# gmh14/tssplat

Hardware: AMD Instinct MI355X
Metric: tetrahedra/sec (energy fwd+bwd) (higher is better)
Workload: dtype f32

## Files before the change

### include/tssplat_amd.h

```cpp
#ifndef TSSPLAT_AMD_H
#define TSSPLAT_AMD_H

#include <stdint.h>

#ifdef __cplusplus
extern "C" {
#endif

typedef struct tsamd_handle tsamd_handle;

typedef enum tsamd_status {
    TSAMD_OK = 0,
    TSAMD_ERR_INVALID_ARGUMENT = 1,
    TSAMD_ERR_BAD_MESH = 2,
    TSAMD_ERR_NO_DEVICE = 3,
    TSAMD_ERR_HIP = 4,
    TSAMD_ERR_IO = 5,
    TSAMD_ERR_TILING = 6,
    TSAMD_ERR_HOST_ONLY = 7
} tsamd_status;

typedef struct tsamd_options {
    int32_t struct_size;
    int32_t device;
// ... 14 lines not shown
    int64_t n_tiles;
    int64_t n_components;
    int64_t total_slots;
    int64_t total_tile_vertices;
    int64_t shared_vertex_copies;
    int64_t finish_vertices;
    int64_t device_bytes;
    int32_t max_slots, max_tile_vertices, block_threads, lds_bytes;
    int32_t slots_per_thread;
    int32_t n_planes;
} tsamd_plan_info;

typedef struct tsamd_partition_info {
    int64_t owned_tets;
    int64_t halo_slots;
    int64_t staged_rows;
    int64_t n_tiles;
    int64_t tile_capacity;
    int64_t min_tiles;
    int64_t cut_components;
    int64_t bisection_components;
    int64_t cut_templates;
    double mean_fill, max_fill;
} tsamd_partition_info;

typedef struct tsamd_tile_view {
    int32_t n_slots, n_owned, s_pad, n_verts, n_excl;
    int64_t stage_off;
    int32_t n_rows;
    int32_t rec_base;
    const uint32_t *planes;
    const uint16_t *row_start;
    const int32_t *gvid;
    const int32_t *vdst;
    const int32_t *slot_tet;
    const float *rest;
} tsamd_tile_view;

const char *tsamd_last_error(void);
const char *tsamd_version(void);
#define TSAMD_ABI_VERSION 3
int32_t tsamd_abi_version(void);

int tsamd_create(const float *rest_xyz, int64_t n_vertices, const int32_t *tets, int64_t n_tets,
                 const tsamd_options *options, tsamd_handle **out);
int tsamd_create_from_veg(const char *path, const tsamd_options *options, tsamd_handle **out);
int tsamd_create_with_operator(const float *rest_xyz, int64_t n_vertices, const int32_t *tets, int64_t n_tets,
                               const int64_t *op_rowptr, const int32_t *op_col, const double *op_val,
                               const tsamd_options *options, tsamd_handle **out);
void tsamd_destroy(tsamd_handle *h);

int64_t tsamd_num_vertices(const tsamd_handle *h);
int64_t tsamd_num_tets(const tsamd_handle *h);
int tsamd_get_plan_info(const tsamd_handle *h, tsamd_plan_info *out);
int tsamd_get_partition_info(const tsamd_handle *h, tsamd_partition_info *out);
int tsamd_get_tile(const tsamd_handle *h, int64_t tile, tsamd_tile_view *out);
int tsamd_get_finish_lists(const tsamd_handle *h, int64_t *n_finish, const int32_t **vid,
                           const int32_t **off, const int32_t **idx);
int tsamd_get_adjacency(const tsamd_handle *h, const int32_t **nbr);

int tsamd_forward(tsamd_handle *h, const float *x_dev, float c1, float c2, int order,
                  void *stream, float *energy_dev);
int tsamd_backward(tsamd_handle *h, const float *x_dev, const float *grad_out_dev, float c1, float c2,
                   int order, void *stream, float *grad_dev);
int tsamd_forward_backward(tsamd_handle *h, const float *x_dev, const float *grad_out_dev, float c1,
                           float c2, int order, void *stream, float *energy_dev, float *grad_dev);
int tsamd_evaluate_dev_coef(tsamd_handle *h, const float *x_dev, const float *grad_out_dev, const float *coef_dev,
                            int order, void *stream, float *energy_dev, float *grad_dev);
typedef struct tsamd_graph tsamd_graph;
int tsamd_graph_create(tsamd_handle *h, const float *x_dev, const float *grad_out_dev, int order, float *energy_dev,
                       float *grad_dev, tsamd_graph **out);
int tsamd_graph_launch(tsamd_graph *graph, float c1, float c2, void *stream);
int tsamd_graph_launch_to(tsamd_graph *graph, float c1, float c2, void *stream, float *energy_copy_dev, float *grad_dev);
void tsamd_graph_destroy(tsamd_graph *graph);

typedef struct tsamd_train_loop tsamd_train_loop;
int64_t tsamd_train_loop_workspace_bytes(int32_t n_iters);
int tsamd_train_loop_create(tsamd_handle *h, float *param_dev, float *grad_dev, float *g1_dev, float *g2_dev, float *energy_ring_dev,
                            void *workspace_dev, int32_t n_iters, tsamd_train_loop **out);
int tsamd_train_loop_launch(tsamd_train_loop *loop, const float *c1, const float *c2, const int32_t *order, float lr, float beta1, float beta2,
                            int64_t first_step, const float *grad_limit, void *stream);
// ... 90 lines not shown
```

### tssplat_amd/_capi.py

```python
from __future__ import annotations

import ctypes as C
import os

from . import _build

_lib = None


class TsamdError(RuntimeError):

    def __init__(self, code: int, message: str):
        super().__init__(f"tssplat_amd error {code}: {message}")
        self.code = code


class Options(C.Structure):
    _fields_ = [
        ("struct_size", C.c_int32),
        ("device", C.c_int32),
        ("lds_budget_bytes", C.c_int32),
        ("max_threads", C.c_int32),
        ("target_owned", C.c_int32),
        ("lane_search_sweeps", C.c_int32),
# ... 4 lines not shown
        ("rebuild_dminv", C.c_int32),
        ("abi_version", C.c_int32),
    ]


class PlanInfo(C.Structure):
    _fields_ = [
        ("n_vertices", C.c_int64), ("n_tets", C.c_int64), ("n_tiles", C.c_int64),
        ("n_components", C.c_int64), ("total_slots", C.c_int64), ("total_tile_vertices", C.c_int64),
        ("shared_vertex_copies", C.c_int64), ("finish_vertices", C.c_int64), ("device_bytes", C.c_int64),
        ("max_slots", C.c_int32), ("max_tile_vertices", C.c_int32), ("block_threads", C.c_int32),
        ("lds_bytes", C.c_int32), ("slots_per_thread", C.c_int32), ("n_planes", C.c_int32),
    ]

    def as_dict(self) -> dict:
        return {k: int(getattr(self, k)) for k, _ in self._fields_}


class PartitionInfo(C.Structure):
    _fields_ = [
        ("owned_tets", C.c_int64), ("halo_slots", C.c_int64), ("staged_rows", C.c_int64), ("n_tiles", C.c_int64),
        ("tile_capacity", C.c_int64), ("min_tiles", C.c_int64), ("cut_components", C.c_int64),
        ("bisection_components", C.c_int64), ("cut_templates", C.c_int64), ("mean_fill", C.c_double), ("max_fill", C.c_double),
    ]


class TileView(C.Structure):
    _fields_ = [
        ("n_slots", C.c_int32), ("n_owned", C.c_int32), ("s_pad", C.c_int32), ("n_verts", C.c_int32),
        ("n_excl", C.c_int32), ("stage_off", C.c_int64), ("n_rows", C.c_int32), ("rec_base", C.c_int32),
        ("planes", C.POINTER(C.c_uint32)), ("row_start", C.POINTER(C.c_uint16)),
        ("gvid", C.POINTER(C.c_int32)), ("vdst", C.POINTER(C.c_int32)), ("slot_tet", C.POINTER(C.c_int32)), ("rest", C.POINTER(C.c_float)),
    ]


ABI_VERSION = 3

SIGNATURES = {
    "tsamd_last_error": (C.c_char_p, []),
    "tsamd_version": (C.c_char_p, []),
    "tsamd_abi_version": (C.c_int32, []),
    "tsamd_create": (C.c_int, [C.c_void_p, C.c_int64, C.c_void_p, C.c_int64, C.POINTER(Options), C.POINTER(C.c_void_p)]),
    "tsamd_create_with_operator": (C.c_int, [C.c_void_p, C.c_int64, C.c_void_p, C.c_int64, C.c_void_p, C.c_void_p, C.c_void_p,
                                             C.POINTER(Options), C.POINTER(C.c_void_p)]),
    "tsamd_create_from_veg": (C.c_int, [C.c_char_p, C.POINTER(Options), C.POINTER(C.c_void_p)]),
    "tsamd_destroy": (None, [C.c_void_p]),
    "tsamd_num_vertices": (C.c_int64, [C.c_void_p]),
    "tsamd_num_tets": (C.c_int64, [C.c_void_p]),
    "tsamd_get_plan_info": (C.c_int, [C.c_void_p, C.POINTER(PlanInfo)]),
    "tsamd_get_partition_info": (C.c_int, [C.c_void_p, C.POINTER(PartitionInfo)]),
    "tsamd_get_tile": (C.c_int, [C.c_void_p, C.c_int64, C.POINTER(TileView)]),
    "tsamd_get_finish_lists": (C.c_int, [C.c_void_p, C.POINTER(C.c_int64), C.POINTER(C.POINTER(C.c_int32)),
                                         C.POINTER(C.POINTER(C.c_int32)), C.POINTER(C.POINTER(C.c_int32))]),
    "tsamd_get_adjacency": (C.c_int, [C.c_void_p, C.POINTER(C.POINTER(C.c_int32))]),
    "tsamd_forward": (C.c_int, [C.c_void_p, C.c_void_p, C.c_float, C.c_float, C.c_int, C.c_void_p, C.c_void_p]),
    "tsamd_backward": (C.c_int, [C.c_void_p, C.c_void_p, C.c_void_p, C.c_float, C.c_float, C.c_int, C.c_void_p,
                                 C.c_void_p]),
    "tsamd_forward_backward": (C.c_int, [C.c_void_p, C.c_void_p, C.c_void_p, C.c_float, C.c_float, C.c_int,
                                         C.c_void_p, C.c_void_p, C.c_void_p]),
    "tsamd_evaluate_dev_coef": (C.c_int, [C.c_void_p, C.c_void_p, C.c_void_p, C.c_void_p, C.c_int, C.c_void_p, C.c_void_p,
                                          C.c_void_p]),
    "tsamd_graph_create": (C.c_int, [C.c_void_p, C.c_void_p, C.c_void_p, C.c_int, C.c_void_p, C.c_void_p, C.POINTER(C.c_void_p)]),
    "tsamd_graph_launch": (C.c_int, [C.c_void_p, C.c_float, C.c_float, C.c_void_p]),
    "tsamd_graph_launch_to": (C.c_int, [C.c_void_p, C.c_float, C.c_float, C.c_void_p, C.c_void_p, C.c_void_p]),
    "tsamd_graph_destroy": (None, [C.c_void_p]),
    "tsamd_read_energy_terms": (C.c_int, [C.c_void_p, C.c_void_p, C.POINTER(C.c_double)]),
    "tsamd_set_timing": (C.c_int, [C.c_void_p, C.c_int]),
    "tsamd_get_timing": (C.c_int, [C.c_void_p, C.POINTER(C.c_double), C.POINTER(C.c_double), C.POINTER(C.c_int64)]),
    "tsamd_scale": (C.c_int, [C.c_void_p, C.c_void_p, C.c_void_p, C.c_int64, C.c_void_p]),
    "tsamd_adam_uniform_step": (C.c_int, [C.c_void_p, C.c_void_p, C.c_void_p, C.c_void_p, C.c_int64, C.c_float, C.c_float,
                                        C.c_float, C.c_int64, C.c_float, C.c_void_p, C.c_void_p]),
    "tsamd_grad_limit_workspace_bytes": (C.c_int64, []),
    "tsamd_grad_limit": (C.c_int, [C.c_void_p, C.c_int64, C.c_float, C.c_float, C.c_void_p, C.c_void_p]),
    "tsamd_train_loop_workspace_bytes": (C.c_int64, [C.c_int32]),
    "tsamd_train_loop_create": (C.c_int, [C.c_void_p, C.c_void_p, C.c_void_p, C.c_void_p, C.c_void_p, C.c_void_p, C.c_void_p, C.c_int32,
                                          C.POINTER(C.c_void_p)]),
# ... 123 lines not shown
```

### tssplat_amd/csrc/capi.cpp

```cpp
#include "../../include/tssplat_amd.h"

#include <hip/hip_runtime_api.h>

#include <algorithm>
#include <cmath>
#include <cstdio>
#include <cstdlib>
#include <cstring>
#include <new>
#include <string>
#include <thread>
#include <vector>

#include "capi_common.h"
#include "kernels.h"
#include "plan.h"

namespace {

thread_local std::string g_err;

int fail(int code, const std::string &msg)
{
    g_err = msg;
    return code;
}

}

namespace tsamd {
int capi_fail(int code, const std::string &msg) { return fail(code, msg); }
}

using tsamd::DeviceGuard;

struct tsamd_handle {
    tsamd::Plan plan;
    bool host_only = true;
    int device = -1;
    int64_t device_bytes = 0;
    tsamd::TileDesc *d_tiles = nullptr;
    uint8_t *d_blob = nullptr;
    int32_t *d_gvid = nullptr, *d_vdst = nullptr, *d_fin_vid = nullptr, *d_fin_off = nullptr;
    float *d_stage = nullptr;
    double *d_partials = nullptr;
    double *d_terms = nullptr;
    float *d_energy_scratch = nullptr;
    bool timing = false;
    std::vector<hipEvent_t> events;
};

struct tsamd_graph {
    tsamd::EvalGraph *g = nullptr;
    int device = -1;
};

namespace {

template <class T>
int upload(T *&dst, const void *src, size_t count, int64_t &bytes)
{
    const size_t nbytes = (count ? count : 1) * sizeof(T);
    TSAMD_HIP(hipMalloc(reinterpret_cast<void **>(&dst), nbytes));
    if (count && src) TSAMD_HIP(hipMemcpy(dst, src, count * sizeof(T), hipMemcpyHostToDevice));
    bytes += int64_t(nbytes);
    return TSAMD_OK;
}

void release(tsamd_handle *h)
{
    if (!h) return;
    if (!h->host_only) {
        DeviceGuard g;
        (void)g.enter(h->device);
        (void)hipFree(h->d_tiles);
        (void)hipFree(h->d_blob);
        (void)hipFree(h->d_gvid);
        (void)hipFree(h->d_fin_vid);
        (void)hipFree(h->d_fin_off);
        (void)hipFree(h->d_vdst);
        (void)hipFree(h->d_stage);
        (void)hipFree(h->d_partials);
        (void)hipFree(h->d_terms);
        (void)hipFree(h->d_energy_scratch);
        for (hipEvent_t e : h->events) (void)hipEventDestroy(e);
    }
    delete h;
}

int to_device(tsamd_handle *h, int device)
{
    int count = 0;
    if (hipGetDeviceCount(&count) != hipSuccess || count <= 0)
        return fail(TSAMD_ERR_NO_DEVICE, "no HIP device is visible (this library has no CPU fallback)");
    if (device < 0) TSAMD_HIP(hipGetDevice(&device));
    if (device >= count) return fail(TSAMD_ERR_INVALID_ARGUMENT, "device ordinal out of range");
    hipDeviceProp_t prop;
    TSAMD_HIP(hipGetDeviceProperties(&prop, device));
    if (size_t(h->plan.lds_bytes) > prop.sharedMemPerBlock && size_t(h->plan.lds_bytes) > prop.maxSharedMemoryPerMultiProcessor)
        return fail(TSAMD_ERR_NO_DEVICE, std::string("device ") + prop.name + " (" + prop.gcnArchName +
                                             ") offers less LDS per workgroup than the plan needs; built for gfx950");
    DeviceGuard g;
// ... 6 lines not shown
    if (tsamd::planes_paired(P.spt) && !P.tiles.empty()) {
        tsamd::RawVector<uint32_t> image(P.blob.size());
        const int64_t T = int64_t(P.tiles.size());
        const int nthr = int(std::max<int64_t>(1, std::min<int64_t>({int64_t(std::thread::hardware_concurrency()), 64, T / 64 + 1})));
        std::vector<std::thread> pool;
        for (int w = 0; w < nthr; ++w)
            pool.emplace_back([&, w]() {
                for (int64_t t = T * w / nthr; t < T * (w + 1) / nthr; ++t) {
                    const tsamd::TileDesc &d = P.tiles[size_t(t)];
                    const size_t b0 = size_t(d.blob_off / 4), b1 = t + 1 < T ? size_t(P.tiles[size_t(t) + 1].blob_off / 4) : P.blob.size();
                    const size_t np = size_t(P.n_planes) * size_t(d.s_pad);
                    tsamd::interleave_tile_planes(P.blob.data() + b0, image.data() + b0, P.n_planes, d.s_pad, P.spt);
                    std::memcpy(image.data() + b0 + np, P.blob.data() + b0 + np, (b1 - b0 - np) * 4);
                }
            });
        for (auto &th : pool) th.join();
        const size_t head = size_t(P.tiles[0].blob_off / 4);
        if (head) std::memcpy(image.data(), P.blob.data(), head * 4);
        if ((rc = upload(h->d_blob, reinterpret_cast<const uint8_t *>(image.data()), image.size() * 4, h->device_bytes))) return rc;
    } else if ((rc = upload(h->d_blob, reinterpret_cast<const uint8_t *>(P.blob.data()), P.blob.size() * 4, h->device_bytes))) {
        return rc;
    }
    if ((rc = upload(h->d_gvid, P.gvid.data(), P.gvid.size(), h->device_bytes))) return rc;
    if ((rc = upload(h->d_vdst, P.vdst.data(), P.vdst.size(), h->device_bytes))) return rc;
    if ((rc = upload(h->d_fin_vid, P.fin_vid.data(), P.fin_vid.size(), h->device_bytes))) return rc;
    if ((rc = upload(h->d_fin_off, P.fin_off.data(), P.fin_off.size(), h->device_bytes))) return rc;
    if ((rc = upload(h->d_stage, nullptr, size_t(P.n_stage) * 3 + 3 , h->device_bytes))) return rc;
    if ((rc = upload(h->d_partials, nullptr, P.tiles.size() * 2, h->device_bytes))) return rc;
    if ((rc = upload(h->d_terms, nullptr, 2, h->device_bytes))) return rc;
    if ((rc = upload(h->d_energy_scratch, nullptr, 1, h->device_bytes))) return rc;
    TSAMD_HIP(hipMemset(h->d_terms, 0, 2 * sizeof(double)));
    {
        const hipError_t ce = tsamd::configure_kernels(P.lds_bytes);
        if (ce == hipErrorInvalidDeviceFunction)
            return fail(TSAMD_ERR_HIP, "a tile kernel of this build has a static LDS object: its dynamic LDS array no longer starts at LDS "
                                       "address 0, which the kernels' absolute LDS addressing relies on (kernels.hip: lds_at)");
        TSAMD_HIP(ce);
    }
    return TSAMD_OK;
}

int create_common(const float *rest, int64_t n, const int32_t *tets, int64_t m, const tsamd_options *o,
                  tsamd_handle **out, const tsamd::ElementOperatorCSR *op = nullptr)
{
    if (!out) return fail(TSAMD_ERR_INVALID_ARGUMENT, "out is null");
    *out = nullptr;
    tsamd_options opt;
    std::memset(&opt, 0, sizeof(opt));
    opt.device = -1;
// ... 76 lines not shown
            return rc;
        }
    }
    *out = h;
    return TSAMD_OK;
}

int check_eval(tsamd_handle *h, const float *x)
{
    if (!h) return fail(TSAMD_ERR_INVALID_ARGUMENT, "handle is null");
    if (h->host_only) return fail(TSAMD_ERR_HOST_ONLY, "handle was created host_only; no device path");
    if (!x && h->plan.n > 0) return fail(TSAMD_ERR_INVALID_ARGUMENT, "x_dev is null");
    return TSAMD_OK;
}

tsamd::EvalArgs eval_args(tsamd_handle *h, const float *x, const float *grad_out, float c1, float c2, int order, float *energy,
                          float *grad, const float *coef)
{
    tsamd::EvalArgs a;
    a.tiles = h->d_tiles;
    a.blob = h->d_blob;
    a.gvid = h->d_gvid;
    a.vdst = h->d_vdst;
    a.fin_vid = h->d_fin_vid;
    a.fin_off = h->d_fin_off;
    a.n_tiles = int64_t(h->plan.tiles.size());
    a.n_finish = int64_t(h->plan.fin_vid.size());
    a.block_threads = h->plan.block_threads;
    a.lds_bytes = h->plan.lds_bytes;
    a.vert_stride = h->plan.vert_stride;
    a.weighted = h->plan.n_planes == tsamd::kPlanesWeighted || h->plan.n_planes == tsamd::kPlanesWeightedSym;
    a.n_planes = h->plan.n_planes;
    a.rebuild = h->plan.n_planes == tsamd::kPlanesRebuild;
    a.spt = h->plan.spt;
    a.x = x;
    a.grad_out = grad_out;
    a.c1 = c1;
    a.c2 = c2;
    a.coef = coef;
    a.order = order;
    a.grad = grad;
    a.stage = h->d_stage;
    a.partials = h->d_partials;
    a.energy = energy;
    a.terms = h->d_terms;
    return a;
}

int evaluate(tsamd_handle *h, const float *x, const float *grad_out, float c1, float c2, int order, void *stream,
             float *energy, float *grad, const float *coef = nullptr)
// ... 74 lines not shown
    out->slots_per_thread = P.spt;
    out->n_planes = P.n_planes;
    return TSAMD_OK;
}

int tsamd_get_partition_info(const tsamd_handle *h, tsamd_partition_info *out)
{
    if (!h || !out) return fail(TSAMD_ERR_INVALID_ARGUMENT, "null argument");
    const tsamd::Plan &P = h->plan;
    std::memset(out, 0, sizeof(*out));
    out->owned_tets = P.m;
    out->halo_slots = P.total_slots - P.m;
    out->staged_rows = P.n_stage;
    out->n_tiles = int64_t(P.tiles.size());
    out->tile_capacity = int64_t(P.block_threads) * P.spt;
    out->min_tiles = out->tile_capacity > 0 ? (P.total_slots + out->tile_capacity - 1) / out->tile_capacity : 0;
    out->cut_components = P.n_cut_components;
    out->bisection_components = P.n_bisection_components;
    out->cut_templates = P.n_cut_templates;
    if (out->n_tiles > 0 && out->tile_capacity > 0) {
        out->mean_fill = double(P.total_slots) / (double(out->n_tiles) * double(out->tile_capacity));
        out->max_fill = double(P.max_slots) / double(out->tile_capacity);
    }
    return TSAMD_OK;
}

int tsamd_get_tile(const tsamd_handle *h, int64_t tile, tsamd_tile_view *out)
{
    if (!h || !out) return fail(TSAMD_ERR_INVALID_ARGUMENT, "null argument");
    const tsamd::Plan &P = h->plan;
    if (tile < 0 || tile >= int64_t(P.tiles.size())) return fail(TSAMD_ERR_INVALID_ARGUMENT, "tile out of range");
    const tsamd::TileDesc &d = P.tiles[size_t(tile)];
    out->n_slots = d.n_slots;
    out->n_owned = d.n_owned;
    out->s_pad = d.s_pad;
    out->n_verts = d.n_verts;
    out->n_excl = d.n_excl;
    out->stage_off = d.stage_off;
    out->n_rows = d.n_rows;
    out->rec_base = d.rec_base;
    out->planes = P.blob.data() + d.blob_off / 4;
    out->row_start = reinterpret_cast<const uint16_t *>(reinterpret_cast<const uint8_t *>(out->planes) + tsamd::tile_rowtab_offset(P.n_planes, d.s_pad));
    out->gvid = P.gvid.data() + d.vert_off;
    out->vdst = P.vdst.data() + d.vert_off;
    out->slot_tet = P.slot_tet.data() + P.slot_base[size_t(tile)];
    out->rest = P.n_planes == tsamd::kPlanesRebuild
                    ? reinterpret_cast<const float *>(reinterpret_cast<const uint8_t *>(out->planes) + tsamd::tile_rest_offset(P.n_planes, d.s_pad))
                    : nullptr;
    return TSAMD_OK;
}

int tsamd_get_finish_lists(const tsamd_handle *h, int64_t *n_finish, const int32_t **vid, const int32_t **off,
                           const int32_t **idx)
{
    if (!h || !n_finish || !vid || !off || !idx) return fail(TSAMD_ERR_INVALID_ARGUMENT, "null argument");
    *n_finish = int64_t(h->plan.fin_vid.size());
    *vid = h->plan.fin_vid.data();
    *off = h->plan.fin_off.data();
    *idx = h->plan.fin_idx.data();
    return TSAMD_OK;
}

int tsamd_get_adjacency(const tsamd_handle *h, const int32_t **nbr)
{
    if (!h || !nbr) return fail(TSAMD_ERR_INVALID_ARGUMENT, "null argument");
    *nbr = h->plan.nbr.data();
    return TSAMD_OK;
}

int tsamd_forward(tsamd_handle *h, const float *x_dev, float c1, float c2, int order, void *stream,
                  float *energy_dev)
{
    if (!energy_dev) return fail(TSAMD_ERR_INVALID_ARGUMENT, "energy_dev is null");
    return evaluate(h, x_dev, nullptr, c1, c2, order, stream, energy_dev, nullptr);
}

int tsamd_backward(tsamd_handle *h, const float *x_dev, const float *grad_out_dev, float c1, float c2, int order,
                   void *stream, float *grad_dev)
{
    if (!grad_dev && h && h->plan.n > 0) return fail(TSAMD_ERR_INVALID_ARGUMENT, "grad_dev is null");
    return evaluate(h, x_dev, grad_out_dev, c1, c2, order, stream, nullptr, grad_dev);
}

int tsamd_forward_backward(tsamd_handle *h, const float *x_dev, const float *grad_out_dev, float c1, float c2,
                           int order, void *stream, float *energy_dev, float *grad_dev)
// ... 210 lines not shown
```

### tssplat_amd/csrc/kernels.h

```cpp
#pragma once

#include <hip/hip_runtime_api.h>

#include <cstdint>

#include "plan.h"

namespace tsamd {

struct EvalArgs {
    const TileDesc *tiles;
    const uint8_t *blob;
    const int32_t *gvid, *vdst;
    const int32_t *fin_vid, *fin_off;
    int64_t n_tiles, n_finish;
    int32_t block_threads, lds_bytes;
    int32_t vert_stride = 0;
    bool rebuild = false;
    bool weighted = false;
    int32_t n_planes = 13;
    int32_t spt = kSlotsPerLane;
    const float *x;
    const float *grad_out;
    float c1, c2;
    const float *coef = nullptr;
    int order;
    float *grad;
    float *stage;
    double *partials;
    float *energy;
    double *terms;
};

hipError_t launch_eval(const EvalArgs &a, hipStream_t stream, hipEvent_t *ev = nullptr);
struct EvalGraph;
hipError_t eval_graph_create(const EvalArgs &a, EvalGraph **out);
hipError_t eval_graph_launch(EvalGraph *g, float c1, float c2, hipStream_t stream, float *energy_copy = nullptr, float *grad = nullptr);
// ... 19 lines not shown
```

### tssplat_amd/csrc/kernels.hip

```cpp
#include <hip/hip_runtime.h>

#include <vector>

#include "kernels.h"

namespace tsamd {
namespace {

constexpr int kWave = 64;

#define SLOT_FENCE() __builtin_amdgcn_sched_barrier(0)
#define STAGE_PRIORITY(n) __builtin_amdgcn_s_setprio(n)
#define UNDEF(x) asm volatile("" : "=v"(x))
typedef uint32_t v4u __attribute__((ext_vector_type(4)));
typedef uint32_t v2u __attribute__((ext_vector_type(2)));

__device__ __forceinline__ float det3(const float *F)
{
    return -F[2] * F[4] * F[6] + F[1] * F[5] * F[6] + F[2] * F[3] * F[7] - F[0] * F[5] * F[7] - F[1] * F[3] * F[8] +
           F[0] * F[4] * F[8];
}

__device__ __forceinline__ void cof3(const float *F, float *C)
{
// ... 542 lines not shown
        };
        if (64 * vb0 < td.n_verts) vertex_sums(vb0, dst_row);
        if (64 * nw < td.n_verts) {
            for (int vb = vb0 + nw; 64 * vb < td.n_verts; vb += nw)
                vertex_sums(vb, 64 * vb + lane < td.n_verts ? g_vdst[td.vert_off + 64 * vb + lane] : 0);
        }
    }
#undef t_own
}

template <bool WITH_GRAD, int BLOCK, int WPE, bool WEIGHTED = false, bool REBUILD = false, int SPT = kSlotsPerLane>
__global__ __launch_bounds__(BLOCK, WPE) void tile_energy_kernel(const KernelArgs a)
{
    const int xcd = blockIdx.x & 7, jb = blockIdx.x >> 3;
    const int tile_end = (xcd + 1) * a.tiles_per_xcd < a.n_tiles ? (xcd + 1) * a.tiles_per_xcd : a.n_tiles;
    const int tile = xcd * a.tiles_per_xcd + jb;
    if (jb >= a.tiles_per_xcd || tile >= tile_end) return;
    const int32_t gv0 = __builtin_nontemporal_load(&as_global(a.gvid)[size_t(tile) * size_t(a.vert_stride) + size_t(int(threadIdx.x) < a.vert_stride ? threadIdx.x : 0)]);
    __builtin_amdgcn_sched_barrier(0);
    tile_body<WITH_GRAD, WEIGHTED, REBUILD, SPT>(a, tile, gv0);
}

struct FinishArgs {
    const int32_t *fin_vid, *fin_off;
    int64_t n_finish;
    const float *stage;
    float *grad;
    const float *grad_out;
    const double *partials;
    int64_t n_tiles;
    float c1, c2;
    const float *coef;
    float *energy;
    double *terms;
    float *energy_copy;
};

template <int T>
__device__ __forceinline__ void energy_reduce(const FinishArgs &a, double *red)
{
    const int tid = threadIdx.x;
    const double2 *part = reinterpret_cast<const double2 *>(a.partials);
    double s = 0.0, b = 0.0;
    int64_t t = tid;
    for (; t + 7 * T < a.n_tiles; t += 8 * T) {
        double2 v[8];
#pragma unroll
// ... 25 lines not shown
        const float c1 = a.coef ? a.coef[0] : a.c1, c2 = a.coef ? a.coef[1] : a.c2;
        const float e = float(double(c1) * red[0] + double(c2) * red[T]);
        a.energy[0] = e;
        if (a.energy_copy) a.energy_copy[0] = e;
    }
}

__global__ __launch_bounds__(1024) void energy_reduce_kernel(const FinishArgs a)
{
    __shared__ double red[2 * 1024];
    energy_reduce<1024>(a, red);
}

#define FIN_LOAD(p) (*(p))
__global__ __launch_bounds__(256) void finish_kernel(const FinishArgs a)
{
    __shared__ double red[2 * 256];
    const int tid = threadIdx.x;
    if (blockIdx.x == 0) {
        if (a.energy) energy_reduce<256>(a, red);
        return;
    }
    const float gscale = a.grad_out ? *a.grad_out : 1.f;
    const int64_t stride = int64_t(gridDim.x - 1) * 256;
    for (int64_t k = int64_t(blockIdx.x - 1) * 256 + tid; k < a.n_finish; k += stride) {
        float gx = 0.f, gy = 0.f, gz = 0.f;
        const int32_t e0 = FIN_LOAD(&a.fin_off[k]), e1 = FIN_LOAD(&a.fin_off[k + 1]);
        constexpr int kRowsAhead = 4;
        {
            float3 r[kRowsAhead];
#pragma unroll
            for (int j = 0; j < kRowsAhead; ++j) {
                const int32_t e = e0 + j < e1 ? e0 + j : (e1 > 0 ? e1 - 1 : 0);
                const float *p = a.stage + size_t(e) * 3;
                r[j] = make_float3(FIN_LOAD(p), FIN_LOAD(p + 1), FIN_LOAD(p + 2));
            }
#pragma unroll
            for (int j = 0; j < kRowsAhead; ++j)
                if (e0 + j < e1) {
                    gx += r[j].x;
                    gy += r[j].y;
                    gz += r[j].z;
                }
        }
        for (int32_t e = e0 + kRowsAhead; e < e1; ++e) {
            const float *r = a.stage + size_t(e) * 3;
            gx += FIN_LOAD(r);
            gy += FIN_LOAD(r + 1);
            gz += FIN_LOAD(r + 2);
        }
        float *g = a.grad + size_t(FIN_LOAD(&a.fin_vid[k])) * 3;
        g[0] = gx * gscale;
        g[1] = gy * gscale;
        g[2] = gz * gscale;
    }
}

__global__ __launch_bounds__(256) void scale_kernel(const float *in, const float *scalar, float *out, int64_t n)
{
    const float s = *scalar;
    if (in == out && s == 1.f) return;
    const int64_t stride = int64_t(gridDim.x) * 256;
    const int64_t n4 = n >> 2;
    const float4 *in4 = reinterpret_cast<const float4 *>(in);
    float4 *out4 = reinterpret_cast<float4 *>(out);
    const bool vec = ((reinterpret_cast<uintptr_t>(in) | reinterpret_cast<uintptr_t>(out)) & 15) == 0;
    if (vec) {
        for (int64_t i = int64_t(blockIdx.x) * 256 + threadIdx.x; i < n4; i += stride) {
            float4 v = in4[i];
            out4[i] = make_float4(v.x * s, v.y * s, v.z * s, v.w * s);
        }
        for (int64_t i = 4 * n4 + int64_t(blockIdx.x) * 256 + threadIdx.x; i < n; i += stride) out[i] = in[i] * s;
    } else {
        for (int64_t i = int64_t(blockIdx.x) * 256 + threadIdx.x; i < n; i += stride) out[i] = in[i] * s;
    }
}

// ... 188 lines not shown
        k.tiles = e.tiles;
        k.blob = e.blob;
        k.gvid = e.gvid;
        k.vdst = e.vdst;
        k.x = e.x;
        k.grad_out = e.grad_out;
        k.grad = e.grad;
        k.stage = e.stage;
        k.partials = e.partials;
        set_coefficients(k, e.c1, e.c2);
        k.coef = e.coef;
        k.order = e.order;
        k.n_tiles = int(e.n_tiles);
        k.tiles_per_xcd = int((e.n_tiles + 7) / 8);
        k.vert_stride = e.vert_stride;
        k.n_planes = e.n_planes;
        r.tile_fn = tile_kernel_for(e.spt, e.block_threads, e.grad != nullptr, e.weighted, e.rebuild);
        if (!r.tile_fn) return hipErrorInvalidConfiguration;
        r.tile_block = dim3(unsigned(e.block_threads));
        r.tile_grid = dim3(unsigned(8 * k.tiles_per_xcd));
        r.tile_lds = size_t(e.lds_bytes);
    }
    FinishArgs &f = r.f;
    f.fin_vid = e.fin_vid;
    f.fin_off = e.fin_off;
    f.n_finish = e.grad ? e.n_finish : 0;
    f.stage = e.stage;
    f.grad = e.grad;
    f.grad_out = e.grad_out;
    f.partials = e.partials;
    f.n_tiles = e.n_tiles;
    f.c1 = e.c1;
    f.c2 = e.c2;
    f.coef = e.coef;
    f.energy = e.energy;
    f.terms = e.terms;
    f.energy_copy = nullptr;
    if (f.n_finish > 0) {
        r.finish_fn = reinterpret_cast<const void *>(&finish_kernel);
        r.finish_grid = dim3(1u + unsigned(grid_for(f.n_finish, 256, 1 << 20)));
        r.finish_block = dim3(256);
    } else if (f.energy) {
        r.finish_fn = reinterpret_cast<const void *>(&energy_reduce_kernel);
        r.finish_grid = dim3(1);
        r.finish_block = dim3(1024);
    }
    return hipSuccess;
}
// ... 279 lines not shown
```

### tssplat_amd/csrc/plan.cpp

```cpp
#include "plan.h"

#include "conflict_opt.h"
#include "partition.h"

#include <algorithm>
#include <atomic>
#include <cmath>
#include <cstdio>
#include <cstdlib>
#include <cstring>
#include <fstream>
#include <functional>
#include <limits>
#include <numeric>
#include <sstream>
#include <chrono>
#include <thread>

namespace tsamd {
namespace {

struct StageTimer {
    bool on = std::getenv("TSAMD_PLAN_TIMING") != nullptr;
    std::chrono::steady_clock::time_point t0 = std::chrono::steady_clock::now();
    void lap(const char *what)
    {
        if (!on) return;
        const auto t1 = std::chrono::steady_clock::now();
// ... 771 lines not shown
    P.block_threads = std::min(max_threads, ((max_quads + 63) / 64) * 64);
    P.blob.resize(size_t(blob_bytes / 4));
    P.gvid.resize(size_t(vert_off));
    P.vdst.resize(size_t(vert_off));
    P.slot_tet.resize(size_t(slot_off));

    std::vector<int32_t> fin_of(static_cast<size_t>(n), -1);
    {
        int64_t entries = 0;
        for (int64_t v = 0; v < n; ++v) {
            int32_t c = vcount[size_t(v)].load(std::memory_order_relaxed);
            if (c == 1) continue;
            fin_of[size_t(v)] = int32_t(P.fin_vid.size());
            P.fin_vid.push_back(int32_t(v));
            P.fin_off.push_back(int32_t(entries));
            entries += c;
            if (entries >= (int64_t(1) << 31)) {
                err = "too many shared vertex copies for 32-bit offsets";
                return ERR_TILING;
            }
        }
        P.fin_off.push_back(int32_t(entries));
        P.fin_idx.assign(size_t(entries), 0);
        std::vector<int32_t> cur(P.fin_off.begin(), P.fin_off.end() - 1);
        for (int64_t t = 0; t < T; ++t) {
            const TileDesc &d = P.tiles[size_t(t)];
            const auto &tv = tile_verts[size_t(t)];
            int64_t j = 0;
            int32_t *vd = P.vdst.data() + d.vert_off;
            for (int32_t i = 0; i < d.n_verts; ++i) {
                const int32_t v = tv[size_t(i)];
                const int32_t k = fin_of[size_t(v)];
                if (k < 0) {
                    vd[i] = v;
                } else {
                    const int32_t row = cur[size_t(k)]++;
                    vd[i] = ~row;
                    P.fin_idx[size_t(d.stage_off + j++)] = row;
                }
            }
            std::fill_n(vd + d.n_verts, size_t(P.vert_stride - d.n_verts), int32_t(0));
        }
    }
    timer.lap("offsets + allocation + finish lists");
    std::atomic<int> singular{0};
    parallel_chunks(T, 2, nthreads, [&](int64_t b, int64_t e, int w) {
        Scratch &S = get_scratch(w);
        std::vector<int32_t> next_rank, copy_of;
        std::vector<int32_t> lane_nb, lane_item_at, lane_tets;
        for (int64_t t = b; t < e; ++t) {
            const TileDesc &d = P.tiles[size_t(t)];
            auto &own = tiles_owned[size_t(t)];
            auto &halo = tile_halo[size_t(t)];
            const auto &tv = tile_verts[size_t(t)];
            const auto &tdeg = tile_vdeg[size_t(t)];
            const int32_t st = S.next();
            copy_of.assign(size_t(d.n_verts), -1);
            next_rank.assign(size_t(d.n_verts), 0);
            for (int32_t i = d.n_verts - 1; i >= 0; --i) {
                const int32_t v = tv[size_t(i)];
                if (S.vert_stamp[v] == st) copy_of[size_t(i)] = S.vert_local[v];
// ... 351 lines not shown
```

### tssplat_amd/csrc/plan.h

```cpp
#pragma once

#include <cstdint>
#include <memory>
#include <string>
#include <utility>
#include <vector>

#ifdef __HIPCC__
#define TSAMD_HOST_DEVICE __host__ __device__
#else
#define TSAMD_HOST_DEVICE
#endif

namespace tsamd {

struct PlanOptions {
    int lds_budget = 0;
    int max_threads = 0;
    int target_owned = 0;
    int num_threads = 0;
    int conflict_aware = 1;
    int lane_search_sweeps = 2;
    int rebuild_dminv = 0;
    int slots_per_lane = 0;
// ... 69 lines not shown
    template <class U, class... Args>
    void construct(U *p, Args &&...args)
    {
        if constexpr (sizeof...(Args) == 0)
            ::new (static_cast<void *>(p)) U;
        else
            ::new (static_cast<void *>(p)) U(std::forward<Args>(args)...);
    }
};
template <class T>
using RawVector = std::vector<T, DefaultInitAllocator<T>>;

struct Plan {
    int64_t n = 0, m = 0;
    int64_t n_components = 0;
    std::vector<int32_t> nbr;
    std::vector<TileDesc> tiles;
    RawVector<uint32_t> blob;
    RawVector<int32_t> gvid;
    RawVector<int32_t> vdst;
    RawVector<int32_t> slot_tet;
    std::vector<int64_t> slot_base;
    std::vector<int32_t> fin_vid, fin_off, fin_idx;
    int64_t n_stage = 0;
    int64_t total_slots = 0, total_tile_verts = 0;
    int64_t n_cut_components = 0, n_bisection_components = 0, n_cut_templates = 0;
    int32_t max_slots = 0, max_verts = 0, block_threads = 64, lds_bytes = 0, spt = kSlotsPerLane;
    int32_t n_planes = kPlanes;
    int32_t vert_stride = 64;
    std::vector<float> op_diag;
    std::vector<float> op_w;
};

struct ElementOperatorCSR {
    const int64_t *rowptr;
    const int32_t *col;
    const double *val;
};

int build_plan(const float *rest, int64_t n, const int32_t *tets, int64_t m, const PlanOptions &opt,
               Plan &plan, std::string &err, const ElementOperatorCSR *op = nullptr);

int build_adjacency(const int32_t *tets, int64_t n, int64_t m, std::vector<int32_t> &nbr, int nthreads,
                    std::string &err);

int read_veg(const char *path, std::vector<float> &rest, std::vector<int32_t> &tets, std::string &err);
// ... 3 lines not shown
```

### tssplat_amd/tet_spheres_ext.py

```python
from __future__ import annotations

import contextlib
import ctypes as C
import os
import sys

import numpy as np
import torch

from . import _capi

__all__ = ["TetSpheres", "forward", "backward", "random_x", "grad_limit"]

_lib = _capi.load()
CPU_ENERGY = os.environ.get("TSSPLAT_AMD_CPU_ENERGY", "0") == "1"
REBUILD_DMINV = {"1": 1, "2": 2}.get(os.environ.get("TSSPLAT_AMD_REBUILD_DMINV", "0"), 0)
print("initializing")


_raw_stream = getattr(torch._C, "_cuda_getCurrentRawStream", None)


def _stream_ptr(device: torch.device) -> int:
    if _raw_stream is not None and device.index is not None:
# ... 82 lines not shown

    def __del__(self):
        try:
            self.close()
        except Exception:
            pass

    def _handle(self):
        if not self._h.value:
            raise RuntimeError("TetSpheres object is empty (construction failed or it was closed)")
        return self._h

    def plan_info(self) -> dict:
        info = _capi.PlanInfo()
        _capi.check(_lib.tsamd_get_plan_info(self._handle(), C.byref(info)))
        out = info.as_dict()
        cut = _capi.PartitionInfo()
        _capi.check(_lib.tsamd_get_partition_info(self._handle(), C.byref(cut)))
        for k, _ in cut._fields_:
            if k != "n_tiles":
                out[k] = getattr(cut, k)
        return out

    def set_timing(self, enable: bool) -> None:
        _capi.check(_lib.tsamd_set_timing(self._handle(), int(enable)))

    def get_timing(self) -> tuple[float, float, int]:
        a, b, n = C.c_double(), C.c_double(), C.c_int64()
        _capi.check(_lib.tsamd_get_timing(self._handle(), C.byref(a), C.byref(b), C.byref(n)))
        return a.value, b.value, n.value

    def energy_terms(self) -> tuple[float, float]:
        out = (C.c_double * 2)()
        _capi.check(_lib.tsamd_read_energy_terms(self._handle(), _stream_ptr(self.device), out))
        return float(out[0]), float(out[1])


def _check_input(x: torch.Tensor, ts: TetSpheres) -> torch.Tensor:
    if not isinstance(x, torch.Tensor):
        raise TypeError("input must be a torch.Tensor")
    if not x.is_cuda:
        raise RuntimeError("tssplat_amd: input must live on the GPU; there is no CPU fallback")
    if ts.device is None or x.device != ts.device:
        raise RuntimeError(f"input is on {x.device} but the TetSpheres object lives on {ts.device}")
    if x.dtype != torch.float32:
        raise RuntimeError("input must be float32")
# ... 71 lines not shown
```

Baseline: 59.88 billion.

## Group shared vertices into patches with strided staging rows for the finish pass

Reorders the staging buffer so vertices shared by the same set of tiles form patches whose rows are interleaved with a stride. The finish kernel then derives each vertex's rows arithmetically from a per-wave patch descriptor via readlane, replacing the per-vertex CSR offset loads, and adjacent lanes read adjacent rows. The aim is fewer index loads and more coalesced reads of the staging buffer when summing boundary gradient contributions. In exchange, plan construction gets a more complex sort and consistency check, and the ABI and introspection APIs grow.

```diff
diff --git a/include/tssplat_amd.h b/include/tssplat_amd.h
--- a/include/tssplat_amd.h
+++ b/include/tssplat_amd.h
@@ -60,6 +60,9 @@
     int64_t bisection_components;
     int64_t cut_templates;
     double mean_fill, max_fill;
+    int64_t patches;
+    double patch_mean_vertices, patch_median_vertices;
+    double tail_share;
 } tsamd_partition_info;
 
 typedef struct tsamd_tile_view {
@@ -77,7 +80,7 @@
 
 const char *tsamd_last_error(void);
 const char *tsamd_version(void);
-#define TSAMD_ABI_VERSION 3
+#define TSAMD_ABI_VERSION 4
 int32_t tsamd_abi_version(void);
 
 int tsamd_create(const float *rest_xyz, int64_t n_vertices, const int32_t *tets, int64_t n_tets,
@@ -95,6 +98,9 @@
 int tsamd_get_tile(const tsamd_handle *h, int64_t tile, tsamd_tile_view *out);
 int tsamd_get_finish_lists(const tsamd_handle *h, int64_t *n_finish, const int32_t **vid,
                            const int32_t **off, const int32_t **idx);
+int tsamd_get_stage_layout(const tsamd_handle *h, int64_t *n_patches, const int32_t **patches, int64_t *n_shared,
+                           const int32_t **patch_vid, int64_t *n_rows, const int32_t **stage_row);
+int tsamd_read_stage(tsamd_handle *h, void *stream, float *rows_host);
 int tsamd_get_adjacency(const tsamd_handle *h, const int32_t **nbr);
 
 int tsamd_forward(tsamd_handle *h, const float *x_dev, float c1, float c2, int order,
diff --git a/tssplat_amd/_capi.py b/tssplat_amd/_capi.py
--- a/tssplat_amd/_capi.py
+++ b/tssplat_amd/_capi.py
@@ -50,6 +50,7 @@
         ("owned_tets", C.c_int64), ("halo_slots", C.c_int64), ("staged_rows", C.c_int64), ("n_tiles", C.c_int64),
         ("tile_capacity", C.c_int64), ("min_tiles", C.c_int64), ("cut_components", C.c_int64),
         ("bisection_components", C.c_int64), ("cut_templates", C.c_int64), ("mean_fill", C.c_double), ("max_fill", C.c_double),
+        ("patches", C.c_int64), ("patch_mean_vertices", C.c_double), ("patch_median_vertices", C.c_double), ("tail_share", C.c_double),
     ]
 
 
@@ -62,7 +63,7 @@
     ]
 
 
-ABI_VERSION = 3
+ABI_VERSION = 4
 
 SIGNATURES = {
     "tsamd_last_error": (C.c_char_p, []),
@@ -80,6 +81,9 @@
     "tsamd_get_tile": (C.c_int, [C.c_void_p, C.c_int64, C.POINTER(TileView)]),
     "tsamd_get_finish_lists": (C.c_int, [C.c_void_p, C.POINTER(C.c_int64), C.POINTER(C.POINTER(C.c_int32)),
                                          C.POINTER(C.POINTER(C.c_int32)), C.POINTER(C.POINTER(C.c_int32))]),
+    "tsamd_get_stage_layout": (C.c_int, [C.c_void_p, C.POINTER(C.c_int64), C.POINTER(C.POINTER(C.c_int32)), C.POINTER(C.c_int64),
+                                         C.POINTER(C.POINTER(C.c_int32)), C.POINTER(C.c_int64), C.POINTER(C.POINTER(C.c_int32))]),
+    "tsamd_read_stage": (C.c_int, [C.c_void_p, C.c_void_p, C.c_void_p]),
     "tsamd_get_adjacency": (C.c_int, [C.c_void_p, C.POINTER(C.POINTER(C.c_int32))]),
     "tsamd_forward": (C.c_int, [C.c_void_p, C.c_void_p, C.c_float, C.c_float, C.c_int, C.c_void_p, C.c_void_p]),
     "tsamd_backward": (C.c_int, [C.c_void_p, C.c_void_p, C.c_void_p, C.c_float, C.c_float, C.c_int, C.c_void_p,
diff --git a/tssplat_amd/csrc/capi.cpp b/tssplat_amd/csrc/capi.cpp
--- a/tssplat_amd/csrc/capi.cpp
+++ b/tssplat_amd/csrc/capi.cpp
@@ -41,7 +41,8 @@
     int64_t device_bytes = 0;
     tsamd::TileDesc *d_tiles = nullptr;
     uint8_t *d_blob = nullptr;
-    int32_t *d_gvid = nullptr, *d_vdst = nullptr, *d_fin_vid = nullptr, *d_fin_off = nullptr;
+    int32_t *d_gvid = nullptr, *d_vdst = nullptr, *d_patch_vid = nullptr, *d_patch_wave = nullptr;
+    tsamd::Plan::Patch *d_patches = nullptr;
     float *d_stage = nullptr;
     double *d_partials = nullptr;
     double *d_terms = nullptr;
@@ -76,8 +77,9 @@
         (void)hipFree(h->d_tiles);
         (void)hipFree(h->d_blob);
         (void)hipFree(h->d_gvid);
-        (void)hipFree(h->d_fin_vid);
-        (void)hipFree(h->d_fin_off);
+        (void)hipFree(h->d_patches);
+        (void)hipFree(h->d_patch_vid);
+        (void)hipFree(h->d_patch_wave);
         (void)hipFree(h->d_vdst);
         (void)hipFree(h->d_stage);
         (void)hipFree(h->d_partials);
@@ -130,9 +132,14 @@
         return rc;
     }
     if ((rc = upload(h->d_gvid, P.gvid.data(), P.gvid.size(), h->device_bytes))) return rc;
-    if ((rc = upload(h->d_vdst, P.vdst.data(), P.vdst.size(), h->device_bytes))) return rc;
-    if ((rc = upload(h->d_fin_vid, P.fin_vid.data(), P.fin_vid.size(), h->device_bytes))) return rc;
-    if ((rc = upload(h->d_fin_off, P.fin_off.data(), P.fin_off.size(), h->device_bytes))) return rc;
+    {
+        tsamd::RawVector<int32_t> image(P.vdst.size());
+        for (size_t i = 0; i < image.size(); ++i) image[i] = P.vdst[i] >= 0 ? P.vdst[i] : ~P.stage_row[size_t(~P.vdst[i])];
+        if ((rc = upload(h->d_vdst, image.data(), image.size(), h->device_bytes))) return rc;
+    }
+    if ((rc = upload(h->d_patches, P.patches.data(), P.patches.size(), h->device_bytes))) return rc;
+    if ((rc = upload(h->d_patch_vid, P.patch_vid.data(), P.patch_vid.size(), h->device_bytes))) return rc;
+    if ((rc = upload(h->d_patch_wave, P.patch_wave.data(), P.patch_wave.size(), h->device_bytes))) return rc;
     if ((rc = upload(h->d_stage, nullptr, size_t(P.n_stage) * 3 + 3 , h->device_bytes))) return rc;
     if ((rc = upload(h->d_partials, nullptr, P.tiles.size() * 2, h->device_bytes))) return rc;
     if ((rc = upload(h->d_terms, nullptr, 2, h->device_bytes))) return rc;
@@ -255,10 +262,11 @@
     a.blob = h->d_blob;
     a.gvid = h->d_gvid;
     a.vdst = h->d_vdst;
-    a.fin_vid = h->d_fin_vid;
-    a.fin_off = h->d_fin_off;
+    a.patches = h->d_patches;
+    a.patch_vid = h->d_patch_vid;
+    a.patch_wave = h->d_patch_wave;
     a.n_tiles = int64_t(h->plan.tiles.size());
-    a.n_finish = int64_t(h->plan.fin_vid.size());
+    a.n_finish = int64_t(h->plan.patch_vid.size());
     a.block_threads = h->plan.block_threads;
     a.lds_bytes = h->plan.lds_bytes;
     a.vert_stride = h->plan.vert_stride;
@@ -379,6 +387,10 @@
         out->mean_fill = double(P.total_slots) / (double(out->n_tiles) * double(out->tile_capacity));
         out->max_fill = double(P.max_slots) / double(out->tile_capacity);
     }
+    out->patches = int64_t(P.patches.size()) - 1;
+    out->patch_mean_vertices = out->patches > 0 ? double(P.patch_vid.size()) / double(out->patches) : 0.0;
+    out->patch_median_vertices = P.patch_g_median;
+    out->tail_share = 0.0;
     return TSAMD_OK;
 }
 
@@ -418,6 +430,32 @@
     return TSAMD_OK;
 }
 
+int tsamd_get_stage_layout(const tsamd_handle *h, int64_t *n_patches, const int32_t **patches, int64_t *n_shared,
+                           const int32_t **patch_vid, int64_t *n_rows, const int32_t **stage_row)
+{
+    if (!h || !n_patches || !patches || !n_shared || !patch_vid || !n_rows || !stage_row) return fail(TSAMD_ERR_INVALID_ARGUMENT, "null argument");
+    static_assert(sizeof(tsamd::Plan::Patch) == 16, "a patch descriptor is four int32");
+    const tsamd::Plan &P = h->plan;
+    *n_patches = int64_t(P.patches.size()) - 1;
+    *patches = reinterpret_cast<const int32_t *>(P.patches.data());
+    *n_shared = int64_t(P.patch_vid.size());
+    *patch_vid = P.patch_vid.data();
+    *n_rows = P.n_stage;
+    *stage_row = P.stage_row.data();
+    return TSAMD_OK;
+}
+
+int tsamd_read_stage(tsamd_handle *h, void *stream, float *rows_host)
+{
+    if (!h || !rows_host) return fail(TSAMD_ERR_INVALID_ARGUMENT, "null argument");
+    if (h->host_only) return fail(TSAMD_ERR_HOST_ONLY, "handle was created host_only; no device path");
+    DeviceGuard g;
+    TSAMD_HIP(g.enter(h->device));
+    TSAMD_HIP(hipStreamSynchronize(static_cast<hipStream_t>(stream)));
+    if (h->plan.n_stage > 0) TSAMD_HIP(hipMemcpy(rows_host, h->d_stage, size_t(h->plan.n_stage) * 3 * sizeof(float), hipMemcpyDeviceToHost));
+    return TSAMD_OK;
+}
+
 int tsamd_get_adjacency(const tsamd_handle *h, const int32_t **nbr)
 {
     if (!h || !nbr) return fail(TSAMD_ERR_INVALID_ARGUMENT, "null argument");
diff --git a/tssplat_amd/csrc/kernels.h b/tssplat_amd/csrc/kernels.h
--- a/tssplat_amd/csrc/kernels.h
+++ b/tssplat_amd/csrc/kernels.h
@@ -12,7 +12,8 @@
     const TileDesc *tiles;
     const uint8_t *blob;
     const int32_t *gvid, *vdst;
-    const int32_t *fin_vid, *fin_off;
+    const Plan::Patch *patches;
+    const int32_t *patch_vid, *patch_wave;
     int64_t n_tiles, n_finish;
     int32_t block_threads, lds_bytes;
     int32_t vert_stride = 0;
diff --git a/tssplat_amd/csrc/kernels.hip b/tssplat_amd/csrc/kernels.hip
--- a/tssplat_amd/csrc/kernels.hip
+++ b/tssplat_amd/csrc/kernels.hip
@@ -588,7 +588,8 @@
 }
 
 struct FinishArgs {
-    const int32_t *fin_vid, *fin_off;
+    const int4 *patches;
+    const int32_t *patch_vid, *patch_wave;
     int64_t n_finish;
     const float *stage;
     float *grad;
@@ -660,37 +661,54 @@
         return;
     }
     const float gscale = a.grad_out ? *a.grad_out : 1.f;
-    const int64_t stride = int64_t(gridDim.x - 1) * 256;
-    for (int64_t k = int64_t(blockIdx.x - 1) * 256 + tid; k < a.n_finish; k += stride) {
+    const int lane = tid & (kWave - 1);
+    const int64_t n_waves = (a.n_finish + kWave - 1) / kWave, wave_stride = int64_t(gridDim.x - 1) * (256 / kWave);
+    for (int64_t w = int64_t(blockIdx.x - 1) * (256 / kWave) + __builtin_amdgcn_readfirstlane(tid / kWave); w < n_waves; w += wave_stride) {
+        const int64_t k = w * kWave + lane;
+        const int32_t p0 = __builtin_amdgcn_readfirstlane(FIN_LOAD(&a.patch_wave[w])), p1 = __builtin_amdgcn_readfirstlane(FIN_LOAD(&a.patch_wave[w + 1]));
+        const int np = p1 - p0 + 1;
+        const int32_t vid = k < a.n_finish ? FIN_LOAD(&a.patch_vid[k]) : 0;
+        const int4 mine = FIN_LOAD(&a.patches[p0 + (lane < np ? lane : 0)]);
+        int32_t first = __builtin_amdgcn_readfirstlane(mine.x), vs = __builtin_amdgcn_readfirstlane(mine.y),
+                g = __builtin_amdgcn_readfirstlane(mine.z), c = __builtin_amdgcn_readfirstlane(mine.w);
+        for (int j = 1; j < np; ++j) {
+            const int32_t fj = __builtin_amdgcn_readlane(mine.x, j), vj = __builtin_amdgcn_readlane(mine.y, j),
+                          gj = __builtin_amdgcn_readlane(mine.z, j), cj = __builtin_amdgcn_readlane(mine.w, j);
+            const bool take = k >= int64_t(vj);
+            first = take ? fj : first, vs = take ? vj : vs, g = take ? gj : g, c = take ? cj : c;
+        }
+        if (k >= a.n_finish) c = 0;
+        const int64_t r0 = int64_t(first) + (k - int64_t(vs));
         float gx = 0.f, gy = 0.f, gz = 0.f;
-        const int32_t e0 = FIN_LOAD(&a.fin_off[k]), e1 = FIN_LOAD(&a.fin_off[k + 1]);
         constexpr int kRowsAhead = 4;
         {
             float3 r[kRowsAhead];
 #pragma unroll
             for (int j = 0; j < kRowsAhead; ++j) {
-                const int32_t e = e0 + j < e1 ? e0 + j : (e1 > 0 ? e1 - 1 : 0);
+                const int64_t e = c > 0 ? r0 + int64_t(j < c ? j : c - 1) * g : 0;
                 const float *p = a.stage + size_t(e) * 3;
                 r[j] = make_float3(FIN_LOAD(p), FIN_LOAD(p + 1), FIN_LOAD(p + 2));
             }
 #pragma unroll
             for (int j = 0; j < kRowsAhead; ++j)
-                if (e0 + j < e1) {
+                if (j < c) {
                     gx += r[j].x;
                     gy += r[j].y;
                     gz += r[j].z;
                 }
         }
-        for (int32_t e = e0 + kRowsAhead; e < e1; ++e) {
-            const float *r = a.stage + size_t(e) * 3;
+        for (int32_t j = kRowsAhead; j < c; ++j) {
+            const float *r = a.stage + size_t(r0 + int64_t(j) * g) * 3;
             gx += FIN_LOAD(r);
             gy += FIN_LOAD(r + 1);
             gz += FIN_LOAD(r + 2);
         }
-        float *g = a.grad + size_t(FIN_LOAD(&a.fin_vid[k])) * 3;
-        g[0] = gx * gscale;
-        g[1] = gy * gscale;
-        g[2] = gz * gscale;
+        if (k < a.n_finish) {
+            float *gp = a.grad + size_t(vid) * 3;
+            gp[0] = gx * gscale;
+            gp[1] = gy * gscale;
+            gp[2] = gz * gscale;
+        }
     }
 }
 
@@ -925,8 +943,9 @@
         r.tile_lds = size_t(e.lds_bytes);
     }
     FinishArgs &f = r.f;
-    f.fin_vid = e.fin_vid;
-    f.fin_off = e.fin_off;
+    f.patches = reinterpret_cast<const int4 *>(e.patches);
+    f.patch_vid = e.patch_vid;
+    f.patch_wave = e.patch_wave;
     f.n_finish = e.grad ? e.n_finish : 0;
     f.stage = e.stage;
     f.grad = e.grad;
diff --git a/tssplat_amd/csrc/plan.cpp b/tssplat_amd/csrc/plan.cpp
--- a/tssplat_amd/csrc/plan.cpp
+++ b/tssplat_amd/csrc/plan.cpp
@@ -4,6 +4,7 @@
 #include "partition.h"
 
 #include <algorithm>
+#include <array>
 #include <atomic>
 #include <cmath>
 #include <cstdio>
@@ -821,7 +822,95 @@
         }
         P.fin_off.push_back(int32_t(entries));
         P.fin_idx.assign(size_t(entries), 0);
+        const int64_t K = int64_t(P.fin_vid.size());
+        const int32_t *fo = P.fin_off.data();
+        std::vector<int32_t> shr(static_cast<size_t>(entries));
+        std::vector<int64_t> tv_base(size_t(T) + 1, 0);
+        for (int64_t t = 0; t < T; ++t) tv_base[size_t(t) + 1] = tv_base[size_t(t)] + int64_t(tile_verts[size_t(t)].size());
+        RawVector<int32_t> tv_row(static_cast<size_t>(tv_base[size_t(T)]));
         std::vector<int32_t> cur(P.fin_off.begin(), P.fin_off.end() - 1);
+        for (int64_t t = 0; t < T; ++t) {
+            const auto &tv = tile_verts[size_t(t)];
+            for (size_t i = 0; i < tv.size(); ++i) {
+                const int32_t k = fin_of[size_t(tv[i])];
+                if (k < 0) continue;
+                tv_row[size_t(tv_base[size_t(t)]) + i] = cur[size_t(k)] - fo[k];
+                shr[size_t(cur[size_t(k)]++)] = int32_t(t);
+            }
+        }
+        auto set_cmp = [&](int32_t a, int32_t b) {
+            const int32_t *pa = shr.data() + fo[a], *ea = shr.data() + fo[a + 1], *pb = shr.data() + fo[b], *eb = shr.data() + fo[b + 1];
+            for (; pa < ea && pb < eb; ++pa, ++pb)
+                if (*pa != *pb) return *pa < *pb ? -1 : 1;
+            return (pa < ea) == (pb < eb) ? 0 : (pb < eb ? -1 : 1);
+        };
+        auto bucket = [&](int64_t k) { return fo[k + 1] > fo[k] ? int64_t(shr[size_t(fo[k])]) + 1 : int64_t(0); };
+        std::vector<int64_t> bstart(size_t(T) + 2, 0);
+        for (int64_t k = 0; k < K; ++k) ++bstart[size_t(bucket(k)) + 1];
+        for (int64_t b = 0; b <= T; ++b) bstart[size_t(b) + 1] += bstart[size_t(b)];
+        std::vector<int32_t> order(static_cast<size_t>(K));
+        {
+            std::vector<int64_t> fill(bstart.begin(), bstart.end() - 1);
+            for (int64_t k = 0; k < K; ++k) order[size_t(fill[size_t(bucket(k))]++)] = int32_t(k);
+        }
+        parallel_chunks(T + 1, 64, nthreads, [&](int64_t b, int64_t e, int) {
+            for (int64_t q = b; q < e; ++q)
+                std::sort(order.begin() + bstart[size_t(q)], order.begin() + bstart[size_t(q) + 1], [&](int32_t x, int32_t y) {
+                    const int c = set_cmp(x, y);
+                    return c != 0 ? c < 0 : x < y;
+                });
+        });
+        std::vector<int32_t> row0(static_cast<size_t>(K)), gsz(static_cast<size_t>(K));
+        P.patch_vid.resize(size_t(K));
+        int64_t row = 0;
+        for (int64_t i = 0; i < K;) {
+            int64_t j = i + 1;
+            while (j < K && set_cmp(order[size_t(i)], order[size_t(j)]) == 0) ++j;
+            const int32_t k0 = order[size_t(i)], g = int32_t(j - i), c = fo[k0 + 1] - fo[k0];
+            P.patches.push_back({int32_t(row), int32_t(i), g, c});
+            for (int64_t q = i; q < j; ++q) {
+                const int32_t k = order[size_t(q)];
+                row0[size_t(k)] = int32_t(row + (q - i));
+                gsz[size_t(k)] = g;
+                P.patch_vid[size_t(q)] = P.fin_vid[size_t(k)];
+            }
+            row += int64_t(c) * g;
+            i = j;
+        }
+        const int64_t n_patches = int64_t(P.patches.size());
+        P.patches.push_back({int32_t(entries), int32_t(K), 0, 0});
+        P.patch_wave.assign(size_t((K + 63) / 64) + 1, int32_t(std::max<int64_t>(0, n_patches - 1)));
+        for (int64_t w = 0, p = 0; 64 * w < K; ++w) {
+            while (P.patches[size_t(p) + 1].vstart <= 64 * w) ++p;
+            P.patch_wave[size_t(w)] = int32_t(p);
+        }
+        if (n_patches > 0) {
+            std::vector<int32_t> gs(static_cast<size_t>(n_patches));
+            for (int64_t p = 0; p < n_patches; ++p) gs[size_t(p)] = P.patches[size_t(p)].g;
+            std::sort(gs.begin(), gs.end());
+            P.patch_g_median = 0.5 * (double(gs[size_t((n_patches - 1) / 2)]) + double(gs[size_t(n_patches / 2)]));
+        }
+        parallel_chunks(T, 16, nthreads, [&](int64_t b, int64_t e, int) {
+            std::vector<std::array<int32_t, 4>> key;
+            for (int64_t t = b; t < e; ++t) {
+                auto &tv = tile_verts[size_t(t)];
+                auto &td = tile_vdeg[size_t(t)];
+                int32_t *tr = tv_row.data() + tv_base[size_t(t)];
+                key.resize(tv.size());
+                for (size_t i = 0; i < tv.size(); ++i) {
+                    const int32_t k = fin_of[size_t(tv[i])];
+                    key[i] = {-td[i], k < 0 ? 1 : 0, k < 0 ? tv[i] : row0[size_t(k)] + tr[i] * gsz[size_t(k)], tv[i]};
+                }
+                std::sort(key.begin(), key.end());
+                for (size_t i = 0; i < tv.size(); ++i) {
+                    td[i] = -key[i][0];
+                    tr[i] = key[i][2];
+                    tv[i] = key[i][3];
+                }
+            }
+        });
+        P.stage_row.assign(size_t(entries), 0);
+        std::copy(P.fin_off.begin(), P.fin_off.end() - 1, cur.begin());
         for (int64_t t = 0; t < T; ++t) {
             const TileDesc &d = P.tiles[size_t(t)];
             const auto &tv = tile_verts[size_t(t)];
@@ -833,9 +922,14 @@
                 if (k < 0) {
                     vd[i] = v;
                 } else {
-                    const int32_t row = cur[size_t(k)]++;
-                    vd[i] = ~row;
-                    P.fin_idx[size_t(d.stage_off + j++)] = row;
+                    const int32_t r = cur[size_t(k)]++;
+                    vd[i] = ~r;
+                    P.fin_idx[size_t(d.stage_off + j++)] = r;
+                    P.stage_row[size_t(r)] = tv_row[size_t(tv_base[size_t(t)]) + size_t(i)];
+                    if (P.stage_row[size_t(r)] != row0[size_t(k)] + (r - fo[k]) * gsz[size_t(k)]) {
+                        err = "internal: a tile vertex's staging row is not its patch's row for that sharer";
+                        return ERR_TILING;
+                    }
                 }
             }
             std::fill_n(vd + d.n_verts, size_t(P.vert_stride - d.n_verts), int32_t(0));
diff --git a/tssplat_amd/csrc/plan.h b/tssplat_amd/csrc/plan.h
--- a/tssplat_amd/csrc/plan.h
+++ b/tssplat_amd/csrc/plan.h
@@ -115,6 +115,14 @@
     RawVector<int32_t> slot_tet;
     std::vector<int64_t> slot_base;
     std::vector<int32_t> fin_vid, fin_off, fin_idx;
+    struct Patch {
+        int32_t first_row, vstart, g, c;
+    };
+    std::vector<Patch> patches;
+    std::vector<int32_t> patch_vid;
+    std::vector<int32_t> patch_wave;
+    std::vector<int32_t> stage_row;
+    double patch_g_median = 0.0;
     int64_t n_stage = 0;
     int64_t total_slots = 0, total_tile_verts = 0;
     int64_t n_cut_components = 0, n_bisection_components = 0, n_cut_templates = 0;
diff --git a/tssplat_amd/tet_spheres_ext.py b/tssplat_amd/tet_spheres_ext.py
--- a/tssplat_amd/tet_spheres_ext.py
+++ b/tssplat_amd/tet_spheres_ext.py
@@ -128,6 +128,23 @@
                 out[k] = getattr(cut, k)
         return out
 
+    def stage_layout(self) -> dict:
+        import numpy as np
+        n_p, n_s, n_r = C.c_int64(), C.c_int64(), C.c_int64()
+        pat, vid, row = C.POINTER(C.c_int32)(), C.POINTER(C.c_int32)(), C.POINTER(C.c_int32)()
+        _capi.check(_lib.tsamd_get_stage_layout(self._handle(), C.byref(n_p), C.byref(pat), C.byref(n_s), C.byref(vid), C.byref(n_r), C.byref(row)))
+
+        def arr(ptr, count, shape):
+            return np.ctypeslib.as_array(ptr, shape=(count,)).copy().reshape(shape) if count else np.zeros(shape, np.int32)
+        return {"patches": arr(pat, 4 * n_p.value, (n_p.value, 4)), "patch_vid": arr(vid, n_s.value, (n_s.value,)),
+                "stage_row": arr(row, n_r.value, (n_r.value,))}
+
+    def read_stage(self):
+        import numpy as np
+        out = np.zeros((max(self.plan_info()["shared_vertex_copies"], 1), 3), np.float32)
+        _capi.check(_lib.tsamd_read_stage(self._handle(), _stream_ptr(self.device), out.ctypes.data))
+        return out[:self.plan_info()["shared_vertex_copies"]]
+
     def set_timing(self, enable: bool) -> None:
         _capi.check(_lib.tsamd_set_timing(self._handle(), int(enable)))
 
```

After: 58.94 billion. 0.984x the previous value.
